# pariasm/bwd-nlkalman

Measured on AMD Instinct MI355X. Metric: Mpix/s per frame (nlkalman-flt, 1080p sigma=20), higher is better.
Workload: dtype f32; 1 GPU; C2: 1920x1080x3 synthetic AWGN sigma=20, FLT1 temporal (deno0 = spatial FLT1 of frame 0, bsic1=NULL), patch 8, defaults of nlkalman_default_params; parallelism=single GPU, mask_order=serial-exact, match_order=exact (the reference's hy, hx, c order)

## Files before the change

bwd-nlkalman_amd/csrc/k_match.h:

```cpp
#pragma once
#include "nlk_common.h"

#include <type_traits>
#ifndef NLK_BM_BLOCK7
#define NLK_BM_BLOCK7 1
#endif
#ifndef NLK_BM_THREADS
#define NLK_BM_THREADS 256
#endif
#define NLK_BM_WAVES (NLK_BM_THREADS / 64)

struct NlkTile {
  int tgx, tgy;
  int bx;
  int ntx, nty;
  int rwp, rh_max;
  int ksel_max;
  int halo;
  int block;
  int threads;
  int order;
};

__device__ __forceinline__ uint32_t nlk_wave_or32(uint32_t v) {
  v |= (uint32_t)__builtin_amdgcn_update_dpp(0, (int)v, 0xB1 , 0xF, 0xF, true);
  v |= (uint32_t)__builtin_amdgcn_update_dpp(0, (int)v, 0x4E , 0xF, 0xF, true);
  v |= (uint32_t)__builtin_amdgcn_update_dpp(0, (int)v, 0x141 , 0xF, 0xF, true);
  v |= (uint32_t)__builtin_amdgcn_update_dpp(0, (int)v, 0x140 , 0xF, 0xF, true);
  const auto a = __builtin_amdgcn_permlane16_swap(v, v, false, false);
  v = a[0] | a[1];
  const auto b = __builtin_amdgcn_permlane32_swap(v, v, false, false);
  return b[0] | b[1];
}
__device__ __forceinline__ uint64_t nlk_wave_or(uint64_t v) {
  return (uint64_t)nlk_wave_or32((uint32_t)v) | ((uint64_t)nlk_wave_or32((uint32_t)(v >> 32)) << 32);
}

template <int PSZ, int CH, int M>
__device__ __forceinline__ void nlk_match_select(const float (&acc)[M], const uint32_t (&wxy)[M], int n, int k,
                                                 int x0, int y0, uint64_t* __restrict__ surv,
                                                 uint32_t* __restrict__ sel, int lane) {
  uint32_t key[M];
  bool ok[M];
  const float norm = (float)(PSZ * PSZ * CH);
#pragma unroll
  for (int m = 0; m < M; ++m) {
    const float q = acc[m] / norm;
    key[m] = __float_as_uint(q > 0.f ? q : 0.f);
    ok[m] = lane + 64 * m < n;
  }

  int kk = k;
  uint64_t alive[M], less[M];
  int nalive = 0;
#pragma unroll
  for (int m = 0; m < M; ++m) {
    alive[m] = __ballot(ok[m]);
    less[m] = 0;
    nalive += __popcll(alive[m]);
  }
#pragma unroll 1
  for (int b = 31; b >= 0 && nalive != kk; --b) {
    uint64_t one[M];
    int cnt0 = 0;
#pragma unroll
    for (int m = 0; m < M; ++m) {
      one[m] = __ballot((key[m] >> b) & 1u);
      cnt0 += __popcll(alive[m] & ~one[m]);
    }
    if (kk > cnt0) {
#pragma unroll
      for (int m = 0; m < M; ++m) {
        less[m] |= alive[m] & ~one[m];
        alive[m] &= one[m];
      }
      kk -= cnt0;
      nalive -= cnt0;
    } else {
#pragma unroll
      for (int m = 0; m < M; ++m) alive[m] &= ~one[m];
      nalive = cnt0;
    }
  }
  int ntie = 0, npos = 0;
  const uint64_t lt_mask = (1ull << lane) - 1ull;
#pragma unroll
  for (int m = 0; m < M; ++m) {
    const uint64_t be = alive[m];
    const int my_tie = ntie + __popcll(be & lt_mask);
    ntie += __popcll(be);
    const bool mine = (be >> lane) & 1ull;
    const bool keep = ((less[m] >> lane) & 1ull) || (mine && my_tie < kk);
    const uint64_t bk = __ballot(keep);
    if (keep) {
      const int pos = npos + __popcll(bk & lt_mask);
      surv[pos] = ((uint64_t)key[m] << 32) | wxy[m];
    }
    npos += __popcll(bk);
  }
  nlk_wave_lds_fence();

  if (k <= 32) {
    const int p = lane & 31, half = lane >> 5, kh = (k + 1) >> 1;
    const uint64_t mine = p < k ? surv[p] : ~0ull;
    const int j0 = half ? kh : 0;
    const int nh = (half ? k : kh) - j0;
    const uint64_t* sp = surv + j0;
    int rank = 0;
    for (int j = 0; j < kh; j += 4) {
      uint64_t sv[4];
#pragma unroll
      for (int u = 0; u < 4; ++u) sv[u] = sp[j + u];
#pragma unroll
      for (int u = 0; u < 4; ++u) rank += (j + u < nh) && sv[u] < mine;
    }
    rank += __shfl_xor(rank, 32, 64);
    if (lane < k) {
      const uint32_t mi = (uint32_t)mine;
      sel[rank] = nlk_pack_xy(x0 + (int)(mi & 0xFFFFu), y0 + (int)(mi >> 16));
    }
  } else {
    for (int base = 0; base < k; base += 64) {
      const int p = base + lane;
      const uint64_t mine = p < k ? surv[p] : ~0ull;
      int rank = 0;
      for (int j = 0; j < k; j += 4) {
        uint64_t sv[4];
#pragma unroll
        for (int u = 0; u < 4; ++u) sv[u] = surv[j + u];
#pragma unroll
        for (int u = 0; u < 4; ++u) rank += (j + u < k) && sv[u] < mine;
      }
      if (p < k) {
        const uint32_t mi = (uint32_t)mine;
        sel[rank] = nlk_pack_xy(x0 + (int)(mi & 0xFFFFu), y0 + (int)(mi >> 16));
      }
    }
  }
  nlk_wave_lds_fence();
}

template <int PSZ, int CH, int M, int ORD = 0>
__device__ __forceinline__ void nlk_match_target(const float* __restrict__ tile, int plane, int rwp,
                                        const float* __restrict__ tgt, int tplane, int trw,
                                        int cbase, int nwx, int n, int k, int x0, int y0,
                                        uint64_t* __restrict__ surv, uint32_t* __restrict__ sel,
                                        int lane) {
  int cq[M];
  uint32_t wxy[M];
  float acc[M];
#pragma unroll
  for (int m = 0; m < M; ++m) {
    const int i = min(lane + 64 * m, n - 1);
    const int wy = i / nwx, wx = i - wy * nwx;
    cq[m] = cbase + wy * rwp + wx;
    wxy[m] = ((uint32_t)wy << 16) | (uint32_t)wx;
    acc[m] = 0.f;
  }
  if constexpr (ORD == 1) {
    constexpr int step = PSZ / 2;
    float sb[2][2][M];
#pragma unroll
    for (int i = 0; i < 4; ++i)
#pragma unroll
      for (int m = 0; m < M; ++m) sb[i >> 1][i & 1][m] = 0.f;
#pragma unroll
    for (int sy = 0; sy < 2; ++sy) {
#pragma unroll 1
      for (int hy = sy * step; hy < (sy + 1) * step; ++hy) {
        const float* trow = tgt + hy * trw;
#pragma unroll
        for (int hx = 0; hx < PSZ; ++hx)
#pragma unroll
          for (int c = 0; c < CH; ++c) {
// ... 10 lines not shown
    for (int m = 0; m < M; ++m) acc[m] = (sb[0][0][m] + sb[0][1][m]) + (sb[1][0][m] + sb[1][1][m]);
    nlk_match_select<PSZ, CH, M>(acc, wxy, n, k, x0, y0, surv, sel, lane);
    return;
  }
#pragma unroll 1
  for (int hy = 0; hy < PSZ; ++hy) {
#pragma clang fp contract(off)
    const float* trow = tgt + hy * trw;
#pragma unroll
    for (int hx = 0; hx < PSZ; ++hx)
#pragma unroll
      for (int c = 0; c < CH; ++c) {
        const float tv = trow[c * tplane + hx];
#pragma unroll
        for (int m = 0; m < M; ++m) {
          const float e = tile[c * plane + cq[m] + hy * rwp + hx] - tv;
          const float e2 = e * e;
          acc[m] = acc[m] + e2;
        }
      }
  }
  nlk_match_select<PSZ, CH, M>(acc, wxy, n, k, x0, y0, surv, sel, lane);
}

#ifndef NLK_BM_SCALAR_TARGET
#define NLK_BM_SCALAR_TARGET 1
#endif
template <int PSZ, int CH, int BX, int M, bool B0, bool B1>
__device__ __forceinline__ void nlk_block_rows(const float* __restrict__ tile, int plane, int rwp, int tbase,
                                               const int (&cq)[M], int ry0, int ry1, float (&acc)[2][BX][M],
                                               const float* __restrict__ timg, int w, size_t npix) {
  constexpr int step = PSZ / 2, UW = (BX - 1) * step + PSZ;
  const float* splane[CH];
#pragma unroll
  for (int c = 0; c < CH; ++c) splane[c] = timg + c * npix;
#pragma unroll 1
  for (int ry = ry0; ry < ry1; ++ry) {
#pragma clang fp contract(off)
    const float* trow = tile + tbase + ry * rwp;
    const int soff = ry * w;
    float tvs[CH][UW];
#pragma unroll
    for (int c = 0; c < CH; ++c) {
      const float* srow = splane[c] + soff;
#pragma unroll
      for (int rx = 0; rx < UW; ++rx) tvs[c][rx] = NLK_BM_SCALAR_TARGET ? srow[rx] : trow[c * plane + rx];
    }
#pragma unroll
    for (int rx = 0; rx < UW; ++rx)
#pragma unroll
      for (int c = 0; c < CH; ++c) {
        const float tv = tvs[c][rx];
#pragma unroll
        for (int m = 0; m < M; ++m) {
          const float e = tile[c * plane + cq[m] + ry * rwp + rx] - tv;
          const float e2 = e * e;
#pragma unroll
          for (int bx = 0; bx < BX; ++bx)
            if (rx >= bx * step && rx < bx * step + PSZ) {
              if (B0) acc[0][bx][m] = acc[0][bx][m] + e2;
              if (B1) acc[1][bx][m] = acc[1][bx][m] + e2;
            }
        }
      }
  }
}
template <int M>
__device__ __forceinline__ void nlk_window_xy(int wsz, int n, int lane, uint32_t (&wxy)[M]) {
  const int nwx = 2 * wsz + 1;
#pragma unroll
  for (int m = 0; m < M; ++m) {
    const int i = min(lane + 64 * m, n - 1);
    const int wy = i / nwx, wx = i - wy * nwx;
    wxy[m] = ((uint32_t)wy << 16) | (uint32_t)wx;
  }
}
template <int PSZ, int CH, int BX, int M>
__device__ __forceinline__ void nlk_match_block(const float* __restrict__ tile, int plane, int rwp, int tbase,
                                                int wsz, int n, int lane, float (&acc)[2][BX][M],
                                                const float* __restrict__ timg, int w, size_t npix) {
  constexpr int step = PSZ / 2;
  const int nwx = 2 * wsz + 1;
  int cq[M];
#pragma unroll
  for (int m = 0; m < M; ++m) {
    const int i = min(lane + 64 * m, n - 1);
    const int wy = i / nwx, wx = i - wy * nwx;
    cq[m] = tbase + (wy - wsz) * rwp + (wx - wsz);
#pragma unroll
    for (int by = 0; by < 2; ++by)
#pragma unroll
      for (int bx = 0; bx < BX; ++bx) acc[by][bx][m] = 0.f;
  }
  nlk_block_rows<PSZ, CH, BX, M, true, false>(tile, plane, rwp, tbase, cq, 0, step, acc, timg, w, npix);
  nlk_block_rows<PSZ, CH, BX, M, true, true>(tile, plane, rwp, tbase, cq, step, PSZ, acc, timg, w, npix);
  nlk_block_rows<PSZ, CH, BX, M, false, true>(tile, plane, rwp, tbase, cq, PSZ, PSZ + step, acc, timg, w, npix);
}

template <int PSZ, int CH, int BX, int M>
__device__ __forceinline__ void nlk_match_block_sum(const float* __restrict__ tile, int plane, int rwp, int tbase,
                                                    int wsz, int n, int lane, float (&acc)[2][BX][M],
                                                    const float* __restrict__ timg, int w, size_t npix) {
  constexpr int step = PSZ / 2, NSX = BX + 1, UW = NSX * step;
  const int nwx = 2 * wsz + 1;
  int cq[M];
  float sb[3][NSX][M];
#pragma unroll
  for (int m = 0; m < M; ++m) {
    const int i = min(lane + 64 * m, n - 1);
    const int wy = i / nwx, wx = i - wy * nwx;
    cq[m] = tbase + (wy - wsz) * rwp + (wx - wsz);
#pragma unroll
    for (int sy = 0; sy < 3; ++sy)
#pragma unroll
      for (int sx = 0; sx < NSX; ++sx) sb[sy][sx][m] = 0.f;
  }
  const float* splane[CH];
#pragma unroll
  for (int c = 0; c < CH; ++c) splane[c] = timg + c * npix;
#pragma unroll
  for (int sy = 0; sy < 3; ++sy) {
#pragma unroll 1
    for (int ry = sy * step; ry < (sy + 1) * step; ++ry) {
      const int soff = ry * w;
      float tvs[CH][UW];
#pragma unroll
      for (int c = 0; c < CH; ++c) {
        const float* srow = splane[c] + soff;
#pragma unroll
        for (int rx = 0; rx < UW; ++rx) tvs[c][rx] = srow[rx];
      }
#pragma unroll
      for (int rx = 0; rx < UW; ++rx)
#pragma unroll
        for (int c = 0; c < CH; ++c) {
          const float tv = tvs[c][rx];
#pragma unroll
          for (int m = 0; m < M; ++m) {
            const float e = tile[c * plane + cq[m] + ry * rwp + rx] - tv;
            sb[sy][rx / step][m] = fmaf(e, e, sb[sy][rx / step][m]);
          }
        }
    }
  }
#pragma unroll
  for (int by = 0; by < 2; ++by)
#pragma unroll
    for (int bx = 0; bx < BX; ++bx)
#pragma unroll
      for (int m = 0; m < M; ++m)
        acc[by][bx][m] = (sb[by][bx][m] + sb[by][bx + 1][m]) + (sb[by + 1][bx][m] + sb[by + 1][bx + 1][m]);
}

template <int STEP = 0>
__device__ __forceinline__ void nlk_match_epilogue(const NlkGeom& g, size_t t, int px, int py, int prev_p,
                                          int k, const uint32_t* __restrict__ sel,
                                          uint32_t* __restrict__ grp,
                                          const uint8_t* __restrict__ vmap,
                                          uint32_t* __restrict__ topk, NlkTarget* __restrict__ tinfo,
                                          uint32_t* __restrict__ gcoords,
                                          uint64_t* __restrict__ marks, int lane) {
  const int step = STEP ? STEP : g.step;
  NlkTarget info = {0, 0, 0, prev_p, {0ull, 0ull}};
  int np0 = 0;
  uint64_t vb[2] = {0ull, 0ull};
  for (int base = 0; base < k; base += 64) {
    const int i = base + lane;
    uint32_t q = 0;
    int v = 0;
    if (i < k) {
      q = sel[i];
      topk[t * g.kmax + i] = q;
      v = prev_p ? vmap[(size_t)nlk_y(q) * g.w + nlk_x(q)] : 0;
    }
    const uint64_t b = __ballot(v);
    if (base < 128) vb[base >> 6] = b;
    const int slot = np0 + __popcll(b & ((1ull << lane) - 1ull));
    if (v && slot < g.ntagg) grp[slot] = q;
    np0 += __popcll(b);
  }
  nlk_wave_lds_fence();

  int nagg, mark;
  if (g.smoother) {
    nagg = min(np0, g.ntagg);
    mark = np0 > 0;
  } else {
    nagg = min(np0 ? np0 : k, g.ntagg);
    mark = !(g.have_prev && np0 == 0);
  }
  uint64_t mbits = 0;
  const int side = 2 * g.R + 1;
  for (int base = 0; base < nagg; base += 64) {
    const int i = base + lane;
    if (i < nagg) {
      const uint32_t q = np0 ? grp[i] : sel[i];
      gcoords[t * g.gstride + i] = q;
      const int dx = nlk_x(q) - px, dy = nlk_y(q) - py;
      if (mark && g.R <= 3 && dx % step == 0 && dy % step == 0) {
        const int di = dx / step, dj = dy / step;
        mbits |= 1ull << ((dj + g.R) * side + di + g.R);
      }
    }
  }
  if (g.smoother && np0 == 0) {
    nagg = 1;
    if (lane == 0) gcoords[t * g.gstride] = nlk_pack_xy(px, py);
  }
  mbits = nlk_wave_or(mbits);
  if (lane == 0) {
    info.nsel = k;
    info.np0 = np0;
    info.nagg = nagg;
    info.flags = prev_p | (mark << 1);
    info.vbits[0] = vb[0]; info.vbits[1] = vb[1];
    tinfo[t] = info;
    marks[t] = mbits;
  }
}

#ifndef NLK_BM7_WAVES
#define NLK_BM7_WAVES 4
#endif
template <int PSZ, int CH, int MAXM, int BX = 4, int ORD = 0>
__global__ void __launch_bounds__(512, MAXM == 7 ? (BX == 2 ? NLK_BM7_WAVES : 3) : ((MAXM == 2 && PSZ == 8) ? 8 : 2))
k_bm_topk(const float* __restrict__ img, const uint8_t* __restrict__ vmap, NlkGeom g,
          NlkTile tl, uint32_t* __restrict__ topk, NlkTarget* __restrict__ tinfo,
          uint32_t* __restrict__ gcoords, uint64_t* __restrict__ marks,
          uint32_t* __restrict__ wide_list, uint32_t* __restrict__ wide_count) {
  extern __shared__ __attribute__((aligned(16))) float smem[];
  const int lane = threadIdx.x & 63;
  const int wave = __builtin_amdgcn_readfirstlane(threadIdx.x >> 6);
  const int nwaves = (int)(blockDim.x >> 6);
  const int tile_id = nlk_xcd_tile(blockIdx.x, tl.ntx * tl.nty);
  if (tile_id >= tl.ntx * tl.nty) return;
  const int ord_y = tile_id / tl.ntx, ord_x = tile_id - ord_y * tl.ntx;
  const int tile_y = ord_y == 0 ? tl.nty - 1 : ord_y - 1;
  const int tile_x = ord_x == 0 ? 0 : (ord_x == 1 ? tl.ntx - 1 : ord_x - 1);
  const int gx0 = tile_x * tl.tgx, gy0 = tile_y * tl.tgy;
  const int cx = min(tl.tgx, g.ngx - gx0), cy = min(tl.tgy, g.ngy - gy0);
  const int wmax = tl.halo;
  constexpr int step = PSZ / 2;

  const int rx0 = max(gx0 * step - wmax, 0);
  const int rx1 = min((gx0 + cx - 1) * step + wmax + PSZ, g.w);
  const int ry0 = max(g.oy + gy0 * step - wmax, 0);
  const int ry1 = min(g.oy + (gy0 + cy - 1) * step + wmax + PSZ, g.h);
  const int rw = rx1 - rx0, rh = ry1 - ry0;
  const int rwp = tl.rwp;
  const int plane = rwp * tl.rh_max;

  float* tile = smem;
  uint64_t* surv_all = (uint64_t*)(tile + ((CH * plane + 1) & ~1));
  uint32_t* sel_all = (uint32_t*)(surv_all + nwaves * tl.ksel_max);
  uint32_t* grp_all = sel_all + nwaves * tl.ksel_max;

  const size_t npix = (size_t)g.w * g.h;
  {
    const int nrows = CH * rh;
    for (int r0 = wave; r0 < nrows; r0 += nwaves * 8) {
      float v0[8], v1[8];
#pragma unroll
      for (int j = 0; j < 8; ++j) {
        const int r = min(r0 + nwaves * j, nrows - 1);
        int c = 0, y = r;
#pragma unroll
        for (int cc = 1; cc < CH; ++cc)
          if (r >= cc * rh) { c = cc; y = r - cc * rh; }
        const float* src = img + c * npix + (size_t)(ry0 + y) * g.w + rx0;
        v0[j] = lane < rw ? src[lane] : 0.f;
        v1[j] = lane + 64 < rw ? src[lane + 64] : 0.f;
      }
#pragma unroll
      for (int j = 0; j < 8; ++j) {
        const int r = r0 + nwaves * j;
        if (r < nrows) {
          int c = 0, y = r;
#pragma unroll
          for (int cc = 1; cc < CH; ++cc)
            if (r >= cc * rh) { c = cc; y = r - cc * rh; }
          float* dst = tile + c * plane + y * rwp;
          if (lane < rw) dst[lane] = v0[j];
          if (lane + 64 < rw) dst[lane + 64] = v1[j];
        }
      }
    }
  }
  __syncthreads();

  int rec_prev = 0;
  if (g.have_prev && lane < cx * cy) {
    const int ty = lane / cx, tx = lane - ty * cx;
    rec_prev = vmap[(size_t)(g.oy + (gy0 + ty) * step) * g.w + (gx0 + tx) * step];
  }
  uint64_t* surv = surv_all + wave * tl.ksel_max;
  uint32_t* sel = sel_all + wave * tl.ksel_max;
  uint32_t* grp = grp_all + wave * g.gstride;

  auto do_target = [&](int tt) {
    const int ty = tt / cx, tx = tt - ty * cx;
    const int gx = gx0 + tx, gy = gy0 + ty;
    const int px = gx * step, py = g.oy + gy * step;
    const size_t t = (size_t)gy * g.ngx + gx;
    const int prev_p = __builtin_amdgcn_readlane(rec_prev, tt);
    int k = prev_p ? g.npt : g.npx;
    NlkTarget info = {0, 0, 0, prev_p, {0ull, 0ull}};
    if (k <= 1) {
      if (g.smoother) {
        info.nagg = 1;
        if (lane == 0) gcoords[t * g.gstride] = nlk_pack_xy(px, py);
      }
      if (lane == 0) { tinfo[t] = info; marks[t] = 0; }
      return;
    }
    const int wsz = (g.smoother || prev_p) ? g.wsz_t : g.wsz_x;
    const int x0 = max(px - wsz, 0), x1 = min(px + wsz, g.w - PSZ) + 1;
    const int y0 = max(py - wsz, 0), y1 = min(py + wsz, g.h - PSZ) + 1;
    const int nwx = x1 - x0, n = nwx * (y1 - y0);
    k = min(k, n);
    const bool in_lds = x0 >= rx0 && x1 - 1 + PSZ <= rx1 && y0 >= ry0 && y1 - 1 + PSZ <= ry1 &&
                        n <= 64 * MAXM;
    if (in_lds) {
      const int cbase = (y0 - ry0) * rwp + (x0 - rx0);
      const float* tl_tgt = tile + (py - ry0) * rwp + (px - rx0);
      if (n <= 128)
        nlk_match_target<PSZ, CH, 2, ORD>(tile, plane, rwp, tl_tgt, plane, rwp, cbase, nwx, n, k, x0,
                                          y0, surv, sel, lane);
      else if (MAXM <= 7 || n <= 448)
        nlk_match_target<PSZ, CH, (MAXM < 7 ? MAXM : 7), ORD>(tile, plane, rwp, tl_tgt, plane, rwp,
                                                              cbase, nwx, n, k, x0, y0, surv,
                                                              sel, lane);
      else
        nlk_match_target<PSZ, CH, MAXM, ORD>(tile, plane, rwp, tl_tgt, plane, rwp, cbase, nwx, n, k,
                                             x0, y0, surv, sel, lane);
    } else {
      if (lane == 0) wide_list[atomicAdd(wide_count, 1u)] = (uint32_t)t;
      return;
    }
    nlk_match_epilogue<PSZ / 2>(g, t, px, py, prev_p, k, sel, grp, vmap, topk, tinfo, gcoords, marks, lane);
    __builtin_amdgcn_wave_barrier();
  };

  if (!tl.block) {
    for (int tt = wave; tt < cx * cy; tt += nwaves) do_target(tt);
    return;
  }
  constexpr int BY = 2;
  const int nbx = (tl.tgx + BX - 1) / BX, nby = (tl.tgy + BY - 1) / BY;
  for (int blk = wave; blk < nbx * nby; blk += nwaves) {
    const int bty = blk / nbx, tx0 = (blk - bty * nbx) * BX, ty0 = bty * BY;
    if (tx0 >= cx || ty0 >= cy) continue;
    bool regular = tx0 + BX <= cx && ty0 + BY <= cy && g.npt > 1 && g.npx > 1;
    int nprev = 0;
    if (regular)
      for (int j = 0; j < BX * BY; ++j)
        nprev += __builtin_amdgcn_readlane(rec_prev, (ty0 + j / BX) * cx + tx0 + j % BX) ? 1 : 0;
    const bool all_t = g.smoother || nprev == BX * BY;
    regular = regular && (all_t || nprev == 0);
    const int wsz = all_t ? g.wsz_t : g.wsz_x;
    const int nwx = 2 * wsz + 1, n = nwx * nwx;
    const int px0 = (gx0 + tx0) * step, py0 = g.oy + (gy0 + ty0) * step;
    constexpr int MB = (MAXM >= 7 && NLK_BM_BLOCK7) ? 7 : 2;
    regular = regular && n <= 64 * MB && wsz <= wmax && px0 - wsz >= rx0 && py0 - wsz >= ry0 &&
              px0 + (BX - 1) * step + wsz + PSZ <= min(rx1, g.w) && py0 + (BY - 1) * step + wsz + PSZ <= min(ry1, g.h);
    if (!regular) {
      for (int j = 0; j < BX * BY; ++j) {
        const int tx = tx0 + j % BX, ty = ty0 + j / BX;
        if (tx < cx && ty < cy) do_target(ty * cx + tx);
      }
      continue;
    }
    auto run_block = [&](auto mtag) {
      constexpr int M = decltype(mtag)::value;
      float acc[2][BX][M];
      if constexpr (ORD == 1)
        nlk_match_block_sum<PSZ, CH, BX, M>(tile, plane, rwp, (py0 - ry0) * rwp + (px0 - rx0), wsz, n, lane, acc,
                                            img + (size_t)py0 * g.w + px0, g.w, (size_t)g.w * g.h);
      else
        nlk_match_block<PSZ, CH, BX, M>(tile, plane, rwp, (py0 - ry0) * rwp + (px0 - rx0), wsz, n, lane, acc,
                                        img + (size_t)py0 * g.w + px0, g.w, (size_t)g.w * g.h);
      int wsz_late = wsz;
      asm volatile("" : "+v"(wsz_late) : "v"(acc[0][0][0]), "v"(acc[1][BX - 1][M - 1]));
      uint32_t wxy[M];
      nlk_window_xy<M>(wsz_late, n, lane, wxy);
#pragma unroll 1
      for (int j = 0; j < BX * BY; ++j) {
        float a2[M];
#pragma unroll
        for (int m = 0; m < M; ++m) a2[m] = 0.f;
#pragma unroll
        for (int by = 0; by < BY; ++by)
#pragma unroll
          for (int bx = 0; bx < BX; ++bx)
            if (j == by * BX + bx) {
#pragma unroll
              for (int m = 0; m < M; ++m) a2[m] = acc[by][bx][m];
            }
        const int tx = tx0 + j % BX, ty = ty0 + j / BX;
        const int gx = gx0 + tx, gy = gy0 + ty;
        const int px = gx * step, py = g.oy + gy * step;
        const size_t t = (size_t)gy * g.ngx + gx;
        const int prev_p = __builtin_amdgcn_readlane(rec_prev, ty * cx + tx);
        const int k = min(prev_p ? g.npt : g.npx, n);
        nlk_match_select<PSZ, CH, M>(a2, wxy, n, k, px - wsz, py - wsz, surv, sel, lane);
        nlk_match_epilogue<PSZ / 2>(g, t, px, py, prev_p, k, sel, grp, vmap, topk, tinfo, gcoords, marks, lane);
        __builtin_amdgcn_wave_barrier();
      }
    };
    if (MB == 2 || n <= 128) run_block(std::integral_constant<int, 2>{});
    else run_block(std::integral_constant<int, MB>{});
  }
}

template <int PSZ, int CH, int MAXM, int ORD = 0>
__global__ void __launch_bounds__(NLK_BM_THREADS)
k_bm_wide(const float* __restrict__ img, const uint8_t* __restrict__ vmap, NlkGeom g, NlkTile tl,
          uint32_t* __restrict__ topk, NlkTarget* __restrict__ tinfo,
          uint32_t* __restrict__ gcoords, uint64_t* __restrict__ marks,
          uint32_t* __restrict__ wide_list, uint32_t* __restrict__ wide_count) {
  extern __shared__ __attribute__((aligned(16))) float smem[];
  constexpr int step = PSZ / 2;
  const int lane = threadIdx.x & 63;
  const int wave = __builtin_amdgcn_readfirstlane(threadIdx.x >> 6);
  const int rwp = tl.rwp, plane = rwp * tl.rh_max;
  const int per_wave = ((CH * plane + 1) & ~1) + ((3 * tl.ksel_max + g.gstride + 1) & ~1);
  float* tile = smem + (size_t)wave * per_wave;
  uint64_t* surv = (uint64_t*)(tile + ((CH * plane + 1) & ~1));
  uint32_t* sel = (uint32_t*)(surv + tl.ksel_max);
  uint32_t* grp = sel + tl.ksel_max;
  const size_t npix = (size_t)g.w * g.h;
  const int count = (int)*wide_count;
  for (int e = blockIdx.x * NLK_BM_WAVES + wave; e < count; e += gridDim.x * NLK_BM_WAVES) {
    const size_t t = wide_list[e];
    const int gy = (int)(t / g.ngx), gx = (int)(t - (size_t)gy * g.ngx);
    const int px = gx * step, py = g.oy + gy * step;
    const int prev_p = g.have_prev ? vmap[(size_t)py * g.w + px] : 0;
    int k = prev_p ? g.npt : g.npx;
    const int wsz = (g.smoother || prev_p) ? g.wsz_t : g.wsz_x;
    const int x0 = max(px - wsz, 0), x1 = min(px + wsz, g.w - PSZ) + 1;
    const int y0 = max(py - wsz, 0), y1 = min(py + wsz, g.h - PSZ) + 1;
    const int nwx = x1 - x0, n = nwx * (y1 - y0);
    k = min(k, n);
    const int rw = x1 - 1 + PSZ - x0, rh = y1 - 1 + PSZ - y0;
    for (int r0 = 0; r0 < CH * rh; r0 += 8) {
      float v[8];
#pragma unroll
      for (int j = 0; j < 8; ++j) {
        const int r = min(r0 + j, CH * rh - 1);
        const int c = r / rh, y = r - c * rh;
        v[j] = lane < rw ? img[c * npix + (size_t)(y0 + y) * g.w + x0 + lane] : 0.f;
      }
#pragma unroll
      for (int j = 0; j < 8; ++j) {
        const int r = r0 + j;
        if (r < CH * rh && lane < rw) {
          const int c = r / rh, y = r - c * rh;
          tile[c * plane + y * rwp + lane] = v[j];
        }
      }
    }
    nlk_wave_lds_fence();
    const float* tl_tgt = tile + (py - y0) * rwp + (px - x0);
    if (n <= 128)
      nlk_match_target<PSZ, CH, 2, ORD>(tile, plane, rwp, tl_tgt, plane, rwp, 0, nwx, n, k, x0, y0, surv,
                                        sel, lane);
    else if (MAXM <= 7 || n <= 448)
      nlk_match_target<PSZ, CH, (MAXM < 7 ? MAXM : 7), ORD>(tile, plane, rwp, tl_tgt, plane, rwp, 0, nwx,
                                                            n, k, x0, y0, surv, sel, lane);
    else
      nlk_match_target<PSZ, CH, MAXM, ORD>(tile, plane, rwp, tl_tgt, plane, rwp, 0, nwx, n, k, x0, y0,
                                           surv, sel, lane);
    nlk_match_epilogue<PSZ / 2>(g, t, px, py, prev_p, k, sel, grp, vmap, topk, tinfo, gcoords, marks, lane);
    __builtin_amdgcn_wave_barrier();
  }
}
```

bwd-nlkalman_amd/csrc/nlk_hip.hip:

```cpp
#include <math.h>
#include <time.h>

#include <algorithm>
#include <mutex>
#include <vector>

namespace nlk_host12 {
#define NLK_HD static inline
#include "k_dct12.h"
#undef NLK_HD
}

#include "k_commit.h"
#include "k_frame.h"
#include "k_match.h"
#include "nlk_internal.h"

char nlk_g_err[512] = "";

namespace {

std::mutex g_live_mu;
std::vector<nlk_ctx*> g_live;

// ... 348 lines not shown
  bool wide = false;
  bool wide0_zeroed = false;
  bool generic = false;
};

static NlkRecView view_rows(nlk_ctx* c, const NlkGeom& g, hipStream_t stream, int r0, int band) {
  const size_t t0 = (size_t)r0 * g.ngx;
  NlkRecView v;
  v.stream = stream;
  v.topk = (uint32_t*)c->topk.p + t0 * g.kmax;
  v.tinfo = (NlkTarget*)c->tinfo.p + t0;
  v.gcoords = (uint32_t*)c->gcoords.p + t0 * g.gstride;
  v.marks = (c->marks_ext ? c->marks_ext : (uint64_t*)c->marks.p) + t0;
  v.wide = (uint32_t*)c->wide.p + t0 + band;
  return v;
}

static NlkGeom band_geom(const NlkGeom& g, int r0, int rows) {
  NlkGeom b = g;
  b.oy = g.oy + r0 * g.step;
  b.ngy = rows;
  return b;
}

static int layout_rows(nlk_ctx* c, const float* cur, const float* prev, const float* basic, float* acc_zero, int w,
                       int h, int ch, int psz, int y0, int y1, int v0, int v1, uint32_t* zero_word = nullptr) {
  const size_t img_floats = (size_t)w * h * ch;
  float* const slab = (float*)c->planes.p;
  if (y1 > y0)
    hipLaunchKernelGGL(ch == 3 ? k_layout<3> : k_layout<0>, dim3((w + 255) / 256, y1 - y0), dim3(256), 0, c->stream, cur, slab, prev,
                       slab + img_floats, basic, slab + 2 * img_floats, (uint8_t*)c->rowok.p, acc_zero, w, h, ch, psz,
                       1, y0, zero_word, (c->layout_diff && prev) ? slab + 3 * img_floats : nullptr);
  if (prev && v1 > v0) {
    if (w % 4 == 0)
      hipLaunchKernelGGL(k_nan_cols4, dim3((w / 4 + 255) / 256, v1 - v0), dim3(256), 0, c->stream,
                         (const uint32_t*)c->rowok.p, (uint32_t*)c->vmap.p, w / 4, h, psz, v0);
    else
      hipLaunchKernelGGL(k_nan_cols, dim3((w + 255) / 256, v1 - v0), dim3(256), 0, c->stream, (const uint8_t*)c->rowok.p,
                         (uint8_t*)c->vmap.p, w, h, psz, v0);
  }
  HIPCHK(c, hipGetLastError());
  return NLK_OK;
}

static int plan_frame(nlk_ctx* c, NlkPlan& pl, const float* cur, const float* prev, const float* basic, int w,
                      int h, int ch, float sigma, const struct nlkalman_params* P, int oy, int ngy,
                      int smoother, int nbands, float* acc_zero = nullptr, bool do_layout = true) {
  int rc = check_images(c, cur, cur, w, h, ch);
  if (rc) return rc;
  if (!P) return fail(c, NLK_EINVAL, "null parameters");
  NLK_USE_DEVICE(c);
  c->lazy_ngx = c->lazy_ngy = 0;
  c->lazy_dst = nullptr;
  NlkGeom& g = pl.g;
  g.w = w; g.h = h; g.ch = ch;
  g.psz = P->patch_sz;
  if (g.psz < 2 || g.psz > 32 || ch * g.psz * g.psz > 4096)
    return fail(c, NLK_EUNSUP, "patch size %d with %d channels not supported (2..32, ch * psz^2 <= 4096)", g.psz, ch);
  g.step = g.psz / 2;
  g.p2 = g.psz * g.psz;
  g.E = g.p2 * ch;
  if (w < g.psz || h < g.psz) return fail(c, NLK_EINVAL, "image smaller than a patch");
  g.ngx = (w - g.psz) / g.step + 1;
  g.oy = oy;
  g.ngy = ngy;
  if (oy < 0 || ngy < 1 || oy + (ngy - 1) * g.step + g.psz > h)
    return fail(c, NLK_EINVAL, "target rows [%d + j*%d, j < %d) leave the %d-row strip", oy,
                g.step, ngy, h);
  g.wsz_x = P->search_sz_x; g.wsz_t = P->search_sz_t;
  g.npx = P->npatches_x; g.npt = P->npatches_t; g.ntagg = P->npatches_tagg;
  if (g.wsz_x < 0 || g.wsz_t < 0 || g.ntagg < 0)
    return fail(c, NLK_EINVAL, "negative search radius or group size (call nlkalman_default_params first)");
  g.have_prev = prev != nullptr;
  g.have_basic = basic != nullptr;
  g.smoother = smoother != 0;
  g.sigma2 = sigma * sigma;
  g.beta_x = P->beta_x; g.beta_t = P->beta_t;
  const int wmax = g.smoother ? g.wsz_t : (g.have_prev ? max(g.wsz_x, g.wsz_t) : g.wsz_x);
  const int wmark = (g.smoother || g.have_prev) ? g.wsz_t : g.wsz_x;
  g.R = wmark / g.step;
  const int ncand = (2 * wmax + 1) * (2 * wmax + 1);
  pl.generic = !(g.psz == 4 || g.psz == 6 || g.psz == 8 || g.psz == 10 || g.psz == 12 || g.psz == 16) ||
               !(ch == 1 || ch == 3) || ncand > 64 * 16 || nlk_set(c->sw.generic_match);
  g.kmax = max(max(g.npx, g.npt), 1);
  const int ngrid = g.ngx * g.ngy;
  const int npix = w * h;
  const int ntagg_alloc = max(g.ntagg, 1);
  g.gstride = ntagg_alloc;

  mark(c, 0);
  {
    const size_t img_floats = (size_t)npix * ch;
    c->layout_diff = g.smoother && prev != nullptr;
    if ((rc = reserve(c, c->planes, sizeof(float) * img_floats * (c->layout_diff ? 4 : (basic ? 3 : (prev ? 2 : 1)))))) return rc;
    pl.img_diff = c->layout_diff ? (const float*)c->planes.p + 3 * img_floats : nullptr;
    c->p_diff = pl.img_diff;
    pl.img_cur = (const float*)c->planes.p;
    pl.img_prev = prev ? pl.img_cur + img_floats : nullptr;
    pl.img_basic = basic ? pl.img_cur + 2 * img_floats : nullptr;
    if (prev && ((rc = reserve(c, c->rowok, npix)) || (rc = reserve(c, c->vmap, npix)))) return rc;
    if ((rc = reserve(c, c->wide, sizeof(uint32_t) * ((size_t)ngrid + nbands)))) return rc;
    if (do_layout) {
      int rc2 = layout_rows(c, cur, prev, basic, acc_zero, w, h, ch, g.psz, 0, h, 0, h, (uint32_t*)c->wide.p);
      if (rc2) return rc2;
      pl.wide0_zeroed = true;
    }
  }
  if ((rc = upload_tables(c, g.psz))) return rc;
  if ((rc = reserve(c, c->topk, sizeof(uint32_t) * (size_t)ngrid * g.kmax)) ||
      (rc = reserve(c, c->tinfo, sizeof(NlkTarget) * (size_t)ngrid)) ||
      (rc = reserve(c, c->gcoords, sizeof(uint32_t) * (size_t)ngrid * ntagg_alloc)) ||
      (rc = reserve(c, c->marks, sizeof(uint64_t) * (size_t)ngrid)) ||
      (rc = reserve(c, c->active, (size_t)ngrid)))
    return rc;
  mark(c, 1);

  pl.img_match = basic ? pl.img_basic : pl.img_cur;
  NlkTile& tl = pl.tl;
  const bool small_grid = (size_t)((g.ngx + 7) / 8) * ((g.ngy + 3) / 4) < 576;
  tl.tgx = nlk_or(c->sw.mtx, small_grid ? 4 : 8);
  tl.tgy = nlk_or(c->sw.mty, small_grid ? 2 : 4);
  tl.threads = NLK_BM_THREADS;
  tl.bx = 4;
  {
    const int halo0 = (g.smoother || g.have_prev) ? g.wsz_t : g.wsz_x;
    const bool tiles84 = tl.tgx == 8 && tl.tgy == 4 && (nlk_set(c->sw.match_block) || !small_grid);
    const int rounds0 = ((2 * halo0 + 1) * (2 * halo0 + 1) + 63) / 64;
    if (nlk_or(c->sw.match_wg8, 0) != 0 && g.psz <= 8 && tiles84) { tl.threads = 512; tl.tgy = 8; }
    else if (nlk_or(c->sw.match_bx2, 1) != 0 && tiles84 && g.psz >= 8 && (rounds0 <= 2 || (g.psz == 8 && rounds0 <= 7))) {
      tl.threads = 512;
      tl.bx = 2;
    }
  }
  tl.ntx = (g.ngx + tl.tgx - 1) / tl.tgx;
  tl.block = nlk_set(c->sw.match_noblock) ? 0 : (nlk_set(c->sw.match_block) ? 1 : !small_grid);
  tl.order = (nlk_or(c->sw.match_order, 0) == 1 && g.psz == 8) ? 1 : 0;
  tl.halo = (g.smoother || g.have_prev) ? g.wsz_t : g.wsz_x;
  {
    const int need = (tl.tgx - 1) * g.step + 2 * tl.halo + g.psz;
    const int wdom = 2 * tl.halo + 1;
    tl.rwp = need + ((wdom - need) % 32 + 32) % 32;
  }
  tl.rh_max = (tl.tgy - 1) * g.step + 2 * tl.halo + g.psz;
  tl.ksel_max = g.kmax;
  auto tile_lds = [&]() {
    return sizeof(float) * ((size_t)ch * tl.rwp * tl.rh_max + 1 + (size_t)(tl.threads / 64) * (3 * tl.ksel_max + ntagg_alloc));
  };
  pl.lds = tile_lds();
  if (pl.lds > 160 * 1024 && tl.threads > NLK_BM_THREADS && tl.tgy == 4) {
    tl.threads = NLK_BM_THREADS;
    tl.bx = 4;
    pl.lds = tile_lds();
  }
  if (pl.lds > 160 * 1024) pl.generic = true;
  pl.wide = !pl.generic && g.have_prev && !g.smoother && g.wsz_x > g.wsz_t;
  const int wdom = 2 * tl.halo + 1;
  pl.maxm = (wdom * wdom + 63) / 64;
  if (pl.wide) {
    NlkTile& tw = pl.tw;
    tw = tl;
    const int need = 2 * g.wsz_x + g.psz, ww = 2 * g.wsz_x + 1;
    tw.halo = g.wsz_x;
    tw.rwp = need + ((ww - need) % 32 + 32) % 32;
    tw.rh_max = need;
    const size_t per_wave = (((size_t)ch * tw.rwp * tw.rh_max + 1) & ~(size_t)1) +
                            ((3 * (size_t)tw.ksel_max + ntagg_alloc + 1) & ~(size_t)1);
    pl.lds_w = sizeof(float) * NLK_BM_WAVES * per_wave;
    if (pl.lds_w > 160 * 1024) { pl.generic = true; pl.wide = false; }
    pl.maxm_w = (ncand + 63) / 64;
  }
  c->p_match = pl.img_match; c->p_cur = pl.img_cur; c->p_prev = pl.img_prev;
  c->last = g;
  c->have_last = true;
  return NLK_OK;
}

static int match_rows(nlk_ctx* c, const NlkPlan& pl, hipStream_t stream, int r0, int rows, int band) {
  const NlkGeom gb = band_geom(pl.g, r0, rows);
  c->rv = view_rows(c, pl.g, stream, r0, band);
  if (pl.generic) return nlk_launch_match_generic(c, gb, pl.img_match);
  NlkTile tl = pl.tl;
  tl.nty = (rows + tl.tgy - 1) / tl.tgy;
  if (pl.wide && !(pl.wide0_zeroed && r0 == 0 && band == 0))
    HIPCHK(c, hipMemsetAsync(c->rv.wide, 0, sizeof(uint32_t), stream));
  int rc = nlk_launch_match(c, gb, tl, pl.lds, pl.img_match, pl.maxm, false);
  if (rc) return rc;
  if (pl.wide) {
    NlkTile tw = pl.tw;
    tw.nty = tl.nty;
    rc = nlk_launch_match(c, gb, tw, pl.lds_w, pl.img_match, pl.maxm_w, true);
  }
  return rc;
}

static int commit_rows(nlk_ctx* c, hipStream_t stream, const uint64_t* marks, uint8_t* active, int ngx, int first,
                       int nrows, int R, int total = 0) {
  total = max(total, first + nrows);
  if (R == 0) {
    HIPCHK(c, hipMemsetAsync(active + (size_t)first * ngx, 1, (size_t)nrows * ngx, stream));
    return NLK_OK;
  }
  if (R == 1 && ngx <= 2048 && !nlk_set(c->sw.commit_wave) && !nlk_set(c->sw.commit_lds) && !nlk_set(c->sw.commit_band)) {
    const int rows_pad = (total + NLK_CR_BATCH - 1) / NLK_CR_BATCH * NLK_CR_BATCH + 3 * NLK_CR_BATCH;
    int rc = reserve(c, c->skew, sizeof(uint32_t) * (size_t)rows_pad * 6 * 64);
    if (rc) return rc;
    uint32_t* planes = (uint32_t*)c->skew.p;
    uint32_t* actbits = planes + (size_t)rows_pad * 4 * 64;
    uint32_t* astate = actbits + (size_t)rows_pad * 64;
    hipLaunchKernelGGL(k_marks_planes1, dim3(8, nrows), dim3(256), 0, stream, marks, planes, ngx, first, (uint32_t*)nullptr);
    hipLaunchKernelGGL(k_mask_commit_rows1, dim3(1), dim3(64), 0, stream, (const uint32_t*)planes, actbits, astate, ngx,
                       first, nrows);
    hipLaunchKernelGGL(k_active_bytes, dim3((ngx + 255) / 256, nrows), dim3(256), 0, stream, (const uint32_t*)actbits,
                       active, ngx, first);
    HIPCHK(c, hipGetLastError());
    return NLK_OK;
  }
  if (R <= 3 && ngx <= 2048 && !nlk_set(c->sw.commit_wave) && !nlk_set(c->sw.commit_lds) && !nlk_set(c->sw.commit_band)) {
    const int np = R + R * (2 * R + 1), pf = 48 / np;
    const int rows_pad = (total + pf - 1) / pf * pf + 3 * pf;
    int rc = reserve(c, c->skew, sizeof(uint32_t) * (size_t)rows_pad * (np + 1 + R) * 64);
    if (rc) return rc;
    uint32_t* planes = (uint32_t*)c->skew.p;
    uint32_t* actbits = planes + (size_t)rows_pad * np * 64;
    uint32_t* astate = actbits + (size_t)rows_pad * 64;
    if (R == 2) {
      hipLaunchKernelGGL(k_marks_planes<2>, dim3(8, nrows), dim3(256), 0, stream, marks, planes, ngx, first, (uint32_t*)nullptr);
      hipLaunchKernelGGL(k_mask_commit_rows<2>, dim3(1), dim3(64), 0, stream, (const uint32_t*)planes, actbits, astate,
                         ngx, first, nrows);
    } else {
      hipLaunchKernelGGL(k_marks_planes<3>, dim3(8, nrows), dim3(256), 0, stream, marks, planes, ngx, first, (uint32_t*)nullptr);
      hipLaunchKernelGGL(k_mask_commit_rows<3>, dim3(1), dim3(64), 0, stream, (const uint32_t*)planes, actbits, astate,
                         ngx, first, nrows);
    }
    hipLaunchKernelGGL(k_active_bytes, dim3((ngx + 255) / 256, nrows), dim3(256), 0, stream, (const uint32_t*)actbits,
                       active, ngx, first);
    HIPCHK(c, hipGetLastError());
    return NLK_OK;
  }
  if (R <= 3 && (first != 0 || !nlk_set(c->sw.commit_lds))) {
    int band = nlk_or(c->sw.commit_band, 1024);
    band = band < 2 * R + 2 ? 2 * R + 2 : (band > 1024 ? 1024 : band);
    auto pre = R == 1 ? k_marks_skew<1> : (R == 2 ? k_marks_skew<2> : k_marks_skew<3>);
    auto kern = R == 1 ? k_mask_commit_wave<1> : (R == 2 ? k_mask_commit_wave<2> : k_mask_commit_wave<3>);
    const int end = first + nrows;
    for (int f = first; f < end;) {
      const int ctx = f == 0 ? 0 : R;
      const int r0 = f - ctx, rows = min(band, end - r0);
      const int threads = ((rows + 63) / 64) * 64;
      const int nsteps = ngx + (R + 1) * (rows - 1);
      const size_t sk_bytes = sizeof(uint32_t) * (size_t)(nsteps + 3 * NLK_CW_PHASE) * threads;
      int rc = reserve(c, c->skew, sk_bytes);
      if (rc) return rc;
      HIPCHK(c, hipMemsetAsync(c->skew.p, 0, sk_bytes, stream));
      hipLaunchKernelGGL(pre, dim3((rows * ngx + 255) / 256), dim3(256), 0, stream, marks + (size_t)r0 * ngx,
                         (uint32_t*)c->skew.p, ngx, rows, threads, (const uint8_t*)active + (size_t)r0 * ngx, ctx);
      hipLaunchKernelGGL(kern, dim3(1), dim3(threads), 0, stream, (const uint32_t*)c->skew.p,
                         active + (size_t)r0 * ngx, ngx, rows, ctx);
      f = r0 + rows;
    }
    HIPCHK(c, hipGetLastError());
    return NLK_OK;
  }
  if (first != 0) return fail(c, NLK_EINVAL, "the LDS / list mask replays take whole grids only");
  const int ngy = nrows, ngrid = ngx * ngy;
  if (R > 3) {
    if (!c->have_last || c->last.ngx != ngx || c->last.ngy != ngy || c->last.R != R ||
        marks != (const uint64_t*)c->marks.p)
      return fail(c, NLK_EUNSUP, "group reach %d grid cells > 3: the mask replay needs the coordinate lists of the "
                  "context's own match phase (row strips across GPUs are limited to reach 3)", R);
    hipLaunchKernelGGL(k_mask_commit_lists, dim3(1), dim3(1024), 0, stream, (const NlkTarget*)c->tinfo.p,
                       (const uint32_t*)c->gcoords.p, c->last.gstride, active, ngx, ngy, R, c->last.step, c->last.oy);
    HIPCHK(c, hipGetLastError());
    return NLK_OK;
  }
  const int rpt = (ngy + 1023) / 1024;
  const int threads = min(1024, ((ngy + 63) / 64) * 64);
  const size_t bits = sizeof(uint32_t) * ((size_t)(ngrid + (R + 1) * ngx + 63) / 32 + 1);
  if (bits > 160 * 1024 || rpt > 4)
    return fail(c, NLK_EUNSUP, "patch grid %dx%d too large for the mask replay", ngx, ngy);
  auto kern = rpt == 1 ? k_mask_commit<1> : (rpt == 2 ? k_mask_commit<2> : k_mask_commit<4>);
  HIPCHK(c, hipFuncSetAttribute((const void*)kern, hipFuncAttributeMaxDynamicSharedMemorySize,
                                (int)bits));
  hipLaunchKernelGGL(kern, dim3(1), dim3(threads), bits, stream, marks, active, ngx, ngy, R);
  HIPCHK(c, hipGetLastError());
  return NLK_OK;
}

static bool chase_selected(const nlk_ctx* c, const NlkGeom& g) {
  return g.R >= 1 && g.R <= 3 && g.ngx <= 2048 && g.psz == 8 && (g.ch == 1 || g.ch == 3) && g.kmax <= 128 && g.gstride <= 128 &&
         !c->deterministic && c->planes.cap < ((size_t)1 << 32) && !nlk_set(c->sw.no_chase) &&
         !nlk_set(c->sw.commit_wave) && !nlk_set(c->sw.commit_lds) && !nlk_set(c->sw.commit_band) &&
         !nlk_set(c->sw.generic_group) && !nlk_set(c->sw.group_packed) && !nlk_set(c->sw.group_dpp);
}

static int chase_prepare(nlk_ctx* c, hipStream_t stream, const uint64_t* marks, int ngx, int nrows, int R) {
  const int np = R == 1 ? 4 : R + R * (2 * R + 1), pf = R == 1 ? NLK_CR_BATCH : 48 / np;
  const int rows_pad = (nrows + pf - 1) / pf * pf + 3 * pf;
  int rc = reserve(c, c->skew, sizeof(uint32_t) * (size_t)rows_pad * np * 64);
  if (rc) return rc;
  const size_t wbytes = sizeof(uint64_t) * (size_t)(nrows + 4 * NLK_CR_BATCH + 1) * 64;
  if (wbytes > c->chase.cap) {
    if ((rc = reserve(c, c->chase, wbytes))) return rc;
    HIPCHK(c, hipMemsetAsync(c->chase.p, 0, c->chase.cap, stream));
  }
  uint32_t* planes = (uint32_t*)c->skew.p;
  uint32_t* gen = (uint32_t*)c->chase.p;
  if (R == 1) hipLaunchKernelGGL(k_marks_planes1, dim3(8, nrows), dim3(256), 0, stream, marks, planes, ngx, 0, gen);
// ... 412 lines not shown
```

Measured before the change: 2279 Mpix/s.

## Stage tile rows with 16-byte loads and cache validity map in LDS

The block-matching kernel's tile staging now has each lane load 4 contiguous floats, packing several rows into one wave pass instead of loading a scalar per lane across 8 rows. When a previous frame exists, the region's validity map is also staged into LDS, provided occupancy does not drop, and the epilogue and rec_prev lookups read it from there instead of issuing scattered global byte loads. Regions wider than 256 columns now fall back to the generic path. The cost is extra LDS use and more complex indexing, with the overlapping tail vector written partially through the skip logic.

```diff
diff --git a/bwd-nlkalman_amd/csrc/k_match.h b/bwd-nlkalman_amd/csrc/k_match.h
--- a/bwd-nlkalman_amd/csrc/k_match.h
+++ b/bwd-nlkalman_amd/csrc/k_match.h
@@ -1,7 +1,11 @@
 #pragma once
 #include "nlk_common.h"
+#include "match_stage.h"
 
 #include <type_traits>
+#ifndef NLK_BM_ONE_TRIP
+#define NLK_BM_ONE_TRIP 1
+#endif
 #ifndef NLK_BM_BLOCK7
 #define NLK_BM_BLOCK7 1
 #endif
@@ -20,6 +24,7 @@
   int block;
   int threads;
   int order;
+  int vlds;
 };
 
 __device__ __forceinline__ uint32_t nlk_wave_or32(uint32_t v) {
@@ -336,6 +341,7 @@
         acc[by][bx][m] = (sb[by][bx][m] + sb[by][bx + 1][m]) + (sb[by + 1][bx][m] + sb[by + 1][bx + 1][m]);
 }
 
+typedef const __attribute__((address_space(3))) uint8_t nlk_lds_u8;
 template <int STEP = 0>
 __device__ __forceinline__ void nlk_match_epilogue(const NlkGeom& g, size_t t, int px, int py, int prev_p,
                                           int k, const uint32_t* __restrict__ sel,
@@ -343,7 +349,9 @@
                                           const uint8_t* __restrict__ vmap,
                                           uint32_t* __restrict__ topk, NlkTarget* __restrict__ tinfo,
                                           uint32_t* __restrict__ gcoords,
-                                          uint64_t* __restrict__ marks, int lane) {
+                                          uint64_t* __restrict__ marks, int lane,
+                                          nlk_lds_u8* __restrict__ vl = nullptr, int vls = 0, int vx0 = 0,
+                                          int vy0 = 0) {
   const int step = STEP ? STEP : g.step;
   NlkTarget info = {0, 0, 0, prev_p, {0ull, 0ull}};
   int np0 = 0;
@@ -355,7 +363,10 @@
     if (i < k) {
       q = sel[i];
       topk[t * g.kmax + i] = q;
-      v = prev_p ? vmap[(size_t)nlk_y(q) * g.w + nlk_x(q)] : 0;
+      if (prev_p) {
+        if (vls) v = vl[(nlk_y(q) - vy0) * vls + (nlk_x(q) - vx0)];
+        else v = vmap[(size_t)nlk_y(q) * g.w + nlk_x(q)];
+      }
     }
     const uint64_t b = __ballot(v);
     if (base < 128) vb[base >> 6] = b;
@@ -403,6 +414,9 @@
   }
 }
 
+#ifndef NLK_BM_STAGE_NB
+#define NLK_BM_STAGE_NB 4
+#endif
 #ifndef NLK_BM7_WAVES
 #define NLK_BM7_WAVES 4
 #endif
@@ -438,8 +452,66 @@
   uint64_t* surv_all = (uint64_t*)(tile + ((CH * plane + 1) & ~1));
   uint32_t* sel_all = (uint32_t*)(surv_all + nwaves * tl.ksel_max);
   uint32_t* grp_all = sel_all + nwaves * tl.ksel_max;
+  const int vls = (NLK_BM_ONE_TRIP && g.have_prev) ? tl.vlds : 0;
+  uint8_t* vl = (uint8_t*)(grp_all + nwaves * g.gstride);
 
   const size_t npix = (size_t)g.w * g.h;
+#if NLK_BM_ONE_TRIP
+  {
+    constexpr int NB = NLK_BM_STAGE_NB, NV = 2;
+    const NlkStageLane sl = nlk_stage_lane(rw, lane);
+    const int nrows = CH * rh, ni = nlk_stage_count(sl, nrows), nv = vls ? nlk_stage_count(sl, rh) : 0;
+    const int wv = nwaves - 1 - wave;
+    const uint8_t* vsrc = (vls ? vmap : (const uint8_t*)img) + (size_t)ry0 * g.w + rx0 + sl.col;
+    auto stage_valid = [&](int i0, uint32_t (&vv)[NV], bool load) {
+#pragma unroll
+      for (int j = 0; j < NV; ++j) {
+        const int y = i0 + nwaves * j < nv ? nlk_stage_row(sl, i0 + nwaves * j, rh) : -1;
+        if (load) {
+          __builtin_memcpy(&vv[j], vsrc + (size_t)max(y, 0) * g.w, 4);
+        } else if (y >= 0) {
+          uint8_t* dst = vl + y * vls + sl.col;
+#pragma unroll
+          for (int e = 0; e < 4; ++e)
+            if (e >= sl.skip) dst[e] = (uint8_t)(vv[j] >> (8 * e));
+        }
+      }
+    };
+    const float* src0 = img + (size_t)ry0 * g.w + rx0 + sl.col;
+    auto stage_rows = [&](int i0, float (&v)[NB][4], bool load) {
+#pragma unroll
+      for (int j = 0; j < NB; ++j) {
+        const int r = i0 + nwaves * j < ni ? nlk_stage_row(sl, i0 + nwaves * j, nrows) : -1;
+        int c = 0, y = max(r, 0);
+#pragma unroll
+        for (int cc = 1; cc < CH; ++cc)
+          if (r >= cc * rh) { c = cc; y = r - cc * rh; }
+        if (load) {
+          __builtin_memcpy(v[j], src0 + c * npix + (size_t)y * g.w, 16);
+        } else if (r >= 0) {
+          float* dst = tile + c * plane + y * rwp + sl.col;
+#pragma unroll
+          for (int e = 0; e < 4; ++e)
+            if (e >= sl.skip) dst[e] = v[j][e];
+        }
+      }
+    };
+    uint32_t vv[NV];
+    float v[NB][4];
+    stage_valid(wv, vv, true);
+    stage_rows(wave, v, true);
+    stage_rows(wave, v, false);
+    stage_valid(wv, vv, false);
+    for (int i0 = wave + nwaves * NB; i0 < ni; i0 += nwaves * NB) {
+      stage_rows(i0, v, true);
+      stage_rows(i0, v, false);
+    }
+    for (int i0 = wv + nwaves * NV; i0 < nv; i0 += nwaves * NV) {
+      stage_valid(i0, vv, true);
+      stage_valid(i0, vv, false);
+    }
+  }
+#else
   {
     const int nrows = CH * rh;
     for (int r0 = wave; r0 < nrows; r0 += nwaves * 8) {
@@ -470,12 +542,18 @@
       }
     }
   }
+#endif
   __syncthreads();
 
   int rec_prev = 0;
   if (g.have_prev && lane < cx * cy) {
     const int ty = lane / cx, tx = lane - ty * cx;
-    rec_prev = vmap[(size_t)(g.oy + (gy0 + ty) * step) * g.w + (gx0 + tx) * step];
+    const int y = g.oy + (gy0 + ty) * step, x = (gx0 + tx) * step;
+    if (vls) {
+      rec_prev = ((nlk_lds_u8*)vl)[(y - ry0) * vls + (x - rx0)];
+    } else {
+      rec_prev = vmap[(size_t)y * g.w + x];
+    }
   }
   uint64_t* surv = surv_all + wave * tl.ksel_max;
   uint32_t* sel = sel_all + wave * tl.ksel_max;
@@ -521,7 +599,8 @@
       if (lane == 0) wide_list[atomicAdd(wide_count, 1u)] = (uint32_t)t;
       return;
     }
-    nlk_match_epilogue<PSZ / 2>(g, t, px, py, prev_p, k, sel, grp, vmap, topk, tinfo, gcoords, marks, lane);
+    nlk_match_epilogue<PSZ / 2>(g, t, px, py, prev_p, k, sel, grp, vmap, topk, tinfo, gcoords, marks, lane,
+                                (nlk_lds_u8*)vl, vls, rx0, ry0);
     __builtin_amdgcn_wave_barrier();
   };
 
@@ -587,7 +666,8 @@
         const int prev_p = __builtin_amdgcn_readlane(rec_prev, ty * cx + tx);
         const int k = min(prev_p ? g.npt : g.npx, n);
         nlk_match_select<PSZ, CH, M>(a2, wxy, n, k, px - wsz, py - wsz, surv, sel, lane);
-        nlk_match_epilogue<PSZ / 2>(g, t, px, py, prev_p, k, sel, grp, vmap, topk, tinfo, gcoords, marks, lane);
+        nlk_match_epilogue<PSZ / 2>(g, t, px, py, prev_p, k, sel, grp, vmap, topk, tinfo, gcoords, marks, lane,
+                                    (nlk_lds_u8*)vl, vls, rx0, ry0);
         __builtin_amdgcn_wave_barrier();
       }
     };
diff --git a/bwd-nlkalman_amd/csrc/match_stage.h b/bwd-nlkalman_amd/csrc/match_stage.h
--- /dev/null
+++ b/bwd-nlkalman_amd/csrc/match_stage.h
@@ -0,0 +1,32 @@
+#pragma once
+
+#ifndef NLK_STAGE_HD
+#if defined(__HIPCC__) || defined(__CUDACC__)
+#define NLK_STAGE_HD __host__ __device__ inline
+#else
+#define NLK_STAGE_HD static inline
+#endif
+#endif
+
+struct NlkStageLane {
+  int sub;
+  int col;
+  int skip;
+  int rpi;
+};
+
+NLK_STAGE_HD NlkStageLane nlk_stage_lane(int rw, int lane) {
+  const int lpr = (rw + 3) >> 2;
+  NlkStageLane s;
+  s.rpi = 64 / lpr;
+  s.sub = lane / lpr;
+  const int c4 = 4 * (lane - s.sub * lpr);
+  s.col = c4 < rw - 4 ? c4 : rw - 4;
+  s.skip = c4 - s.col;
+  return s;
+}
+NLK_STAGE_HD int nlk_stage_count(const NlkStageLane& s, int nrows) { return (nrows + s.rpi - 1) / s.rpi; }
+NLK_STAGE_HD int nlk_stage_row(const NlkStageLane& s, int i, int nrows) {
+  const int r = i * s.rpi + s.sub;
+  return (s.sub < s.rpi && r < nrows) ? r : -1;
+}
diff --git a/bwd-nlkalman_amd/csrc/nlk_hip.hip b/bwd-nlkalman_amd/csrc/nlk_hip.hip
--- a/bwd-nlkalman_amd/csrc/nlk_hip.hip
+++ b/bwd-nlkalman_amd/csrc/nlk_hip.hip
@@ -524,7 +524,17 @@
     tl.bx = 4;
     pl.lds = tile_lds();
   }
+  tl.vlds = 0;
+  if (NLK_BM_ONE_TRIP && g.have_prev) {
+    const size_t vrow = (size_t)((tl.tgx - 1) * g.step + 2 * tl.halo + g.psz + 3) & ~(size_t)3;
+    const size_t with = pl.lds + vrow * tl.rh_max, cu = 160 * 1024;
+    if (with <= cu && cu / with == cu / pl.lds) {
+      tl.vlds = (int)vrow;
+      pl.lds = with;
+    }
+  }
   if (pl.lds > 160 * 1024) pl.generic = true;
+  if (NLK_BM_ONE_TRIP && (tl.tgx - 1) * g.step + 2 * tl.halo + g.psz > 256) pl.generic = true;
   pl.wide = !pl.generic && g.have_prev && !g.smoother && g.wsz_x > g.wsz_t;
   const int wdom = 2 * tl.halo + 1;
   pl.maxm = (wdom * wdom + 63) / 64;
```

Result: no change. 2299 Mpix/s, median of 6 (+0.9%).
